# Vandermode/ELD

Measured on AMD Instinct MI355X. Metric: raw megapixels/sec (noise-synth + U-Net step), higher is better.
Workload: dtype f32; 1 GPU; BASELINE.json configs[1]: full ELD noise model (PGRU, SonyA7S2 params) on 4x1424x2128 packed raw + U-Net fp32 train step (fwd, L1, bwd, Adam), 8 frames per GPU; images_per_gpu=8, global_batch=8, parallelism=dp1

## Files before the change

eld_amd/csrc/conv.h:

```cpp
#pragma once
#include "common.h"

typedef float f32x16 __attribute__((ext_vector_type(16)));
typedef float f32x2 __attribute__((ext_vector_type(2)));
typedef __bf16 bf16x2_hw __attribute__((ext_vector_type(2)));

enum ConvMode { CONV_3X3 = 0, CONV_1X1 = 1, CONV_GATHER2X2 = 2 };
enum ConvEpi { EPI_FWD = 0, EPI_CONVT_FWD = 1, EPI_GRAD = 2 };

typedef unsigned short bf16_t;
enum ConvDtype { DT_F32 = 0, DT_BF16 = 1 };

struct ConvArgs {
    const void* in0;
    const void* in1;
    int C0, C1;
    const void* wp;
    int N, H, W;
    int Nout;
    int epi;
    const float* bias;
    int lrelu;
    void* out0;
    void* out1;
// ... 253 lines not shown
    const int full = tiles_x * BH, band = id / full, off = id - band * full;
    int bh = tiles_y - band * BH;
    if (bh > BH) bh = BH;
    tx = off / bh;
    ty = band * BH + (off - tx * bh);
}
int eld_tile_band();
enum { XCD_GEMM = 1, XCD_WGRAD8 = 2, XCD_WGRAD = 4, XCD_X3D = 8, XCD_X3W = 16, XCD_BF16 = 32, XCD_IGEMM = 64 };
int eld_xcd_mask();

struct WgradArgs {
    const void* g;
    int CA;
    const void* x0;
    const void* x1;
    int C0, C1;
    int N, H, W;
    float* part;
    float* bpart;
    float* xbpart;
    int CBp;
    int psplit;
    int tiles_x, tiles_y;
    int vp;
    int dtype;
    int algo;
    int wgrad8;
    int xcd;
    int band;
    const float* amax_g; const float* amax_x0; const float* amax_x1;
};

int launch_wgrad(const WgradArgs& a, int mode, hipStream_t st);
bool wgrad8_shape(int CA, int CBp, int& COB, int& JB, int& TH, int& TWo, bool bf16 = false);
int wgrad8_ntiles(int CA, int CBp, int N, int H, int W, bool bf16);
bool wgradt8_takes(int CA, int CB);
int wgradt8_ntiles(int N, int H, int W);
int launch_wgrad_reduce(const float* part, const float* bpart, float* wgrad, float* bgrad, int psplit, int T, int CA,
                        int CBp, int CBr, hipStream_t st, int bias_n = 0);
```

eld_amd/csrc/conv_wgrad.hip:

```cpp
#include <stdlib.h>
#include "conv.h"

#define TW 32
#define JB 32

typedef __bf16 bf16x8 __attribute__((ext_vector_type(8)));
typedef short s16x4 __attribute__((ext_vector_type(4)));
typedef int i32x4_t __attribute__((ext_vector_type(4)));
typedef _Float16 half8 __attribute__((ext_vector_type(8)));

enum { ALG_F32 = 0, ALG_BFM = 1, ALG_X3 = 2, ALG_H2 = 3 };

template <typename T, int MODE, int WCO, int TH, int ALG>
__global__ __launch_bounds__(256, 2) void wgrad_kernel(const WgradArgs a) {
    constexpr bool BFM = ALG == ALG_BFM, X3 = ALG == ALG_X3, H2 = ALG == ALG_H2;
    static_assert(!(X3 || H2) || sizeof(T) == 4, "x3 / h2: fp32 inputs");
    constexpr int ES = sizeof(T);
    constexpr int EPU = 16 / ES;
    constexpr int LES = X3 ? 6 : (BFM ? 2 : 4);
    constexpr int TAPS = MODE == CONV_3X3 ? 9 : 4;
    constexpr int WPIX = 4 / WCO;
    constexpr int COB = 32 * WCO;
    constexpr int TPIX = TH * TW;
    constexpr int PW = TPIX / WPIX;
// ... 270 lines not shown
                const int row = (i & 3) + 8 * (i >> 2) + 4 * hi;
                a.part[pbase + ((size_t)t * a.CA + i0 + wco * 32 + row) * a.CBp + j0 + m] = H2 ? acc[t][i] * (1.0f / sc_g) * (1.0f / sc_x) : acc[t][i];
            }
        }
    }
    if (a.bpart && jb == 0) {
        red[wave * 64 + lane] = bsum;
        __syncthreads();
        if (tid < COB) {
            const int wc = tid / 32, mm = tid % 32;
            float s = 0.f;
            for (int wp = 0; wp < WPIX; ++wp) s += red[(wp * WCO + wc) * 64 + mm] + red[(wp * WCO + wc) * 64 + 32 + mm];
            a.bpart[(size_t)ps * a.CA + i0 + tid] = H2 ? s * (1.0f / sc_g) : s;
        }
    }
    if constexpr (XSUM) {
        if (xsum_on) {
            __syncthreads();
            float* r = lds;
#pragma unroll
            for (int e = 0; e < EPU; ++e) r[tid * EPU + e] = xs[e];
            __syncthreads();
            if (tid < JB) {
                constexpr int PARTS = JB / EPU;
                const int part = tid / EPU, comp = tid % EPU;
                float s = 0.f;
                for (int k = 0; k < 256 / PARTS; ++k) s += r[(k * PARTS + part) * EPU + comp];
                a.xbpart[(size_t)ps * a.CBp + j0 + tid] = s;
            }
        }
    }
}

template <typename T, int WCO, int WCI, int WPIX, int TH, int TWT, int STREAM = 0>
__global__ __launch_bounds__(512, 2) void wgrad8_kernel(const WgradArgs a) {
    constexpr int ES = sizeof(T), EPU = 16 / ES, NPC = ES == 4 ? 3 : 1, XQ = 32 / EPU;
    static_assert(WCO * WCI * WPIX == 8, "8 waves");
    constexpr int THREADS = 512, TAPS = 9;
    constexpr int COB = 32 * WCO, JBK = 32 * WCI, TPIX = TH * TWT, PW = TPIX / WPIX, KSB = PW / 16;
    static_assert(TWT == 8 || TWT == 16 || TWT == 32, "tile width");
    static_assert(PW % 16 == 0 && PW >= 16, "a wave's pixel slice is a whole number of 16-pixel k-steps");
    constexpr int X_PIX = (TH + 2) * (TWT + 2);
    constexpr int GBLK = TPIX * 32 + (ES == 4 ? 32 : 0);
    constexpr int GPL = GBLK * WCO, XPL = X_PIX * JBK;
    constexpr int G_Q = COB / EPU, G_UNITS = TPIX * G_Q, G_IT = G_UNITS / THREADS;
    static_assert(G_UNITS % THREADS == 0 && THREADS % G_Q == 0, "a thread stages the same channel quad of G in every iteration");
    constexpr int X_UNITS1 = X_PIX * XQ, X_IT = (X_UNITS1 + THREADS - 1) / THREADS;
    extern __shared__ __attribute__((aligned(16))) float lds[];
    bf16_t* ldsG = reinterpret_cast<bf16_t*>(lds);
    bf16_t* ldsX = ldsG + NPC * GPL;

    const int tid = threadIdx.x, lane = tid & 63, wave = tid >> 6;
    const int m = lane & 31, hi = lane >> 5;
    const int wco = wave % WCO, wci = (wave / WCO) % WCI, wpix = wave / (WCO * WCI);
    const int IB = a.CA / COB, JBn = a.CBp / JBK;
    int bid = xcd_block(a.xcd);
    const int jb = bid % JBn; bid /= JBn;
    const int ib = bid % IB;
    const int ps = bid / IB;
    const int i0 = ib * COB, j0 = jb * JBK;
    const bool do_bias = a.bpart != nullptr && jb == 0;

    f32x16 acc[TAPS];
#pragma unroll
    for (int t = 0; t < TAPS; ++t)
#pragma unroll
        for (int i = 0; i < 16; ++i) acc[t][i] = 0.f;
    float4 bsum4 = make_float4(0.f, 0.f, 0.f, 0.f), bsum4b = make_float4(0.f, 0.f, 0.f, 0.f);

    const int ntiles = a.tiles_x * a.tiles_y;
    const int VP = a.vp;
    const bool seam = VP % TH != 0;
    constexpr unsigned OOB = 0xFFFFFFF0u;
    constexpr int G_STEP = THREADS / G_Q;
    const int g_part = tid % G_Q, g_lp0 = tid / G_Q;
    const int g_px0 = g_lp0 % TWT, g_py0 = g_lp0 / TWT;
    const unsigned g_off0 = (unsigned)(g_px0 * a.CA + i0 + g_part * EPU) * (unsigned)ES;
    const int g_lds0 = ((g_part * EPU) >> 5) * GBLK + g_lp0 * 32 + ((g_part * EPU) & 31);
    auto g_pxy = [&](int it, int& dpx, int& dpy) {
        if (G_STEP >= TWT) { dpx = 0; dpy = it * (G_STEP / TWT); }
        else { dpx = (it * G_STEP) % TWT; dpy = (it * G_STEP) / TWT; }
    };
    const int x_part = (int)((unsigned)tid % (unsigned)XQ);
    int x_hyx[X_IT];
#pragma unroll
    for (int it = 0; it < X_IT; ++it) {
        const int hp = (int)((unsigned)(tid + it * THREADS) / (unsigned)XQ);
        const int hy = hp / (TWT + 2);
        x_hyx[it] = (hy << 8) | (hp - hy * (TWT + 2));
    }
    auto x_alive = [&](int it) { return (it + 1) * THREADS <= X_UNITS1 || (int)((unsigned)(tid + it * THREADS) / (unsigned)XQ) < X_PIX; };
    const char* xs[WCI]; int xC[WCI], xc0[WCI];
#pragma unroll
    for (int cb = 0; cb < WCI; ++cb) {
        const int c = j0 + cb * 32;
        if (c < a.C0) { xs[cb] = static_cast<const char*>(a.x0); xC[cb] = a.C0; xc0[cb] = c; }
        else if (c < a.C0 + a.C1) { xs[cb] = static_cast<const char*>(a.x1); xC[cb] = a.C1; xc0[cb] = c - a.C0; }
        else { xs[cb] = nullptr; xC[cb] = 32; xc0[cb] = 0; }
    }
    float4 rg[G_IT], rx[WCI][X_IT];
    const size_t g_img = (size_t)a.H * a.W * a.CA * ES;
    const unsigned g_rowc = (unsigned)(g_py0 * a.W * a.CA) * (unsigned)ES;
    auto load_tile = [&](int tile) {
        int ty, tx;
        band_tile(tile, a.tiles_x, a.tiles_y, a.band, ty, tx);
        const int v0 = ty * TH, x0 = tx * TWT;
        const int img0 = v0 / VP, vrel = v0 - img0 * VP;
        const int wrem = a.W - x0;
        if (!seam || VP - vrel > TH) {
            const __amdgpu_buffer_rsrc_t rs_g = __builtin_amdgcn_make_buffer_rsrc((void*)(static_cast<const char*>(a.g) + (size_t)img0 * g_img), 0, (int)g_img, 0x00020000);
            const int gbase = (vrel * a.W + x0) * a.CA * ES;
#pragma unroll
            for (int it = 0; it < G_IT; ++it) {
                int dpx, dpy;
                g_pxy(it, dpx, dpy);
                const unsigned off = g_off0 + g_rowc + (unsigned)((dpy * a.W + dpx) * a.CA) * (unsigned)ES;
                rg[it] = __builtin_bit_cast(float4, __builtin_amdgcn_raw_buffer_load_b128(rs_g, g_px0 + dpx < wrem ? (int)off : (int)OOB, gbase, 0));
            }
#pragma unroll
            for (int cb = 0; cb < WCI; ++cb) {
                const size_t x_img = (size_t)a.H * a.W * xC[cb] * ES;
                const __amdgpu_buffer_rsrc_t rs_x = __builtin_amdgcn_make_buffer_rsrc((void*)(xs[cb] ? xs[cb] + (size_t)img0 * x_img : nullptr), 0, xs[cb] ? (int)x_img : 0, 0x00020000);
#pragma unroll
                for (int it = 0; it < X_IT; ++it) {
                    const int gy = vrel - 1 + (x_hyx[it] >> 8), gx = x0 - 1 + (x_hyx[it] & 255);
                    const bool ok = x_alive(it) && (unsigned)gy < (unsigned)a.H && (unsigned)gx < (unsigned)a.W;
                    const unsigned off = ok ? (unsigned)((gy * a.W + gx) * xC[cb] + xc0[cb] + x_part * EPU) * (unsigned)ES : OOB;
                    rx[cb][it] = __builtin_bit_cast(float4, __builtin_amdgcn_raw_buffer_load_b128(rs_x, (int)off, 0, 0));
                }
            }
            return;
        }
        const int nimg = a.N - img0 < 2 ? a.N - img0 : 2;
        const int lim0 = a.H - vrel, nxt = VP - vrel;
        const __amdgpu_buffer_rsrc_t rs_g = __builtin_amdgcn_make_buffer_rsrc((void*)(static_cast<const char*>(a.g) + (size_t)img0 * g_img), 0, (int)(g_img * nimg), 0x00020000);
        const unsigned gb0 = (unsigned)((vrel * a.W + x0) * a.CA) * (unsigned)ES;
        const unsigned gb1 = (unsigned)(((a.H - nxt) * a.W + x0) * a.CA) * (unsigned)ES;
#pragma unroll
        for (int it = 0; it < G_IT; ++it) {
            int dpx, dpy;
            g_pxy(it, dpx, dpy);
            const int r = g_py0 + dpy;
            const bool second = r >= nxt;
            const bool ok = (r < lim0 || (second && r - nxt < a.H)) && g_px0 + dpx < wrem;
            const unsigned off = (second ? gb1 : gb0) + g_off0 + g_rowc + (unsigned)((dpy * a.W + dpx) * a.CA) * (unsigned)ES;
            rg[it] = __builtin_bit_cast(float4, __builtin_amdgcn_raw_buffer_load_b128(rs_g, ok ? (int)off : (int)OOB, 0, 0));
        }
#pragma unroll
        for (int cb = 0; cb < WCI; ++cb) {
            const size_t x_img = (size_t)a.H * a.W * xC[cb] * ES;
            const __amdgpu_buffer_rsrc_t rs_x = __builtin_amdgcn_make_buffer_rsrc((void*)(xs[cb] ? xs[cb] + (size_t)img0 * x_img : nullptr), 0, xs[cb] ? (int)(x_img * nimg) : 0, 0x00020000);
#pragma unroll
            for (int it = 0; it < X_IT; ++it) {
                const int r = (x_hyx[it] >> 8) - 1, gx = x0 - 1 + (x_hyx[it] & 255);
                const bool second = r >= nxt;
                const int wrow = second ? a.H + r - nxt : vrel + r;
                const bool rok = second ? r - nxt < a.H : (unsigned)(vrel + r) < (unsigned)a.H;
                const bool ok = x_alive(it) && rok && (unsigned)gx < (unsigned)a.W;
                const unsigned off = ok ? (unsigned)((wrow * a.W + gx) * xC[cb] + xc0[cb] + x_part * EPU) * (unsigned)ES : OOB;
                rx[cb][it] = __builtin_bit_cast(float4, __builtin_amdgcn_raw_buffer_load_b128(rs_x, (int)off, 0, 0));
            }
        }
    };
    auto put3 = [&](bf16_t* d, int plane_elems, const float4& raw) {
        if constexpr (ES == 2) { *reinterpret_cast<float4*>(d) = raw; return; }
        const unsigned x0 = __float_as_uint(raw.x), x1 = __float_as_uint(raw.y), x2 = __float_as_uint(raw.z), x3 = __float_as_uint(raw.w);
        const float r0 = raw.x - __uint_as_float(x0 & 0xFFFF0000u), r1 = raw.y - __uint_as_float(x1 & 0xFFFF0000u);
        const float r2 = raw.z - __uint_as_float(x2 & 0xFFFF0000u), r3 = raw.w - __uint_as_float(x3 & 0xFFFF0000u);
        const unsigned y0 = __float_as_uint(r0), y1 = __float_as_uint(r1), y2 = __float_as_uint(r2), y3 = __float_as_uint(r3);
        const unsigned z0 = __float_as_uint(r0 - __uint_as_float(y0 & 0xFFFF0000u)), z1 = __float_as_uint(r1 - __uint_as_float(y1 & 0xFFFF0000u));
        const unsigned z2 = __float_as_uint(r2 - __uint_as_float(y2 & 0xFFFF0000u)), z3 = __float_as_uint(r3 - __uint_as_float(y3 & 0xFFFF0000u));
        auto hp = [](unsigned lo, unsigned hi_) { return __builtin_amdgcn_perm(hi_, lo, 0x07060302u); };
        *reinterpret_cast<uint2*>(d) = make_uint2(hp(x0, x1), hp(x2, x3));
        *reinterpret_cast<uint2*>(d + plane_elems) = make_uint2(hp(y0, y1), hp(y2, y3));
        *reinterpret_cast<uint2*>(d + 2 * plane_elems) = make_uint2(hp(z0, z1), hp(z2, z3));
    };
    auto store_tile = [&]() {
#pragma unroll
        for (int it = 0; it < G_IT; ++it) {
            put3(ldsG + g_lds0 + it * G_STEP * 32, GPL, rg[it]);
            if (do_bias) {
                if constexpr (ES == 4) { bsum4.x += rg[it].x; bsum4.y += rg[it].y; bsum4.z += rg[it].z; bsum4.w += rg[it].w; }
                else {
                    const uint4 q = __builtin_bit_cast(uint4, rg[it]);
                    const float4 lo = unpack_bf4(make_uint2(q.x, q.y)), hi4 = unpack_bf4(make_uint2(q.z, q.w));
                    bsum4.x += lo.x; bsum4.y += lo.y; bsum4.z += lo.z; bsum4.w += lo.w;
                    bsum4b.x += hi4.x; bsum4b.y += hi4.y; bsum4b.z += hi4.z; bsum4b.w += hi4.w;
                }
            }
        }
#pragma unroll
        for (int cb = 0; cb < WCI; ++cb)
#pragma unroll
            for (int it = 0; it < X_IT; ++it)
                if (x_alive(it)) put3(ldsX + (cb * X_PIX + (int)((unsigned)(tid + it * THREADS) / (unsigned)XQ)) * 32 + x_part * EPU, XPL, rx[cb][it]);
    };

    const int gi = lane & 15, gg = lane >> 4;
    constexpr bool ROWSHARE = STREAM == 2;
    static_assert(!ROWSHARE || (NPC == 3 && TWT == 8 && WPIX == 1 && TH % 2 == 0), "row-shared fragments: fp32, 8-pixel-wide tiles, one pixel slice");
    constexpr int HS = TH / 2;
    const int lq0 = ROWSHARE ? HS * TWT * hi + (gi >> 2) : wpix * PW + 8 * hi + (gi >> 2);
    const int pyq = lq0 / TWT, pxq = lq0 - pyq * TWT;
    const bf16_t* gq = ldsG + wco * GBLK + lq0 * 32 + (gg & 1) * 16 + (gi & 3) * 4;
    const bf16_t* xq = ldsX + (wci * X_PIX + pyq * (TWT + 2) + pxq) * 32 + (gg & 1) * 16 + (gi & 3) * 4;
    auto tr8 = [](const bf16_t* p0) {
        const s16x4 lo = __builtin_amdgcn_ds_read_tr16_b64_v4i16((__attribute__((address_space(3))) s16x4*)p0);
        const s16x4 hi4 = __builtin_amdgcn_ds_read_tr16_b64_v4i16((__attribute__((address_space(3))) s16x4*)(p0 + 4 * 32));
        return __builtin_bit_cast(bf16x8, __builtin_shufflevector(lo, hi4, 0, 1, 2, 3, 4, 5, 6, 7));
    };

    if (ps < ntiles) load_tile(ps);
    for (int tile = ps; tile < ntiles; tile += a.psplit) {
        __syncthreads();
        store_tile();
        __syncthreads();
        if (tile + a.psplit < ntiles) load_tile(tile + a.psplit);
        if constexpr (ROWSHARE) {
            constexpr int GI[6] = {0, 1, 2, 0, 1, 0};
            constexpr int XI[6] = {2, 1, 0, 1, 0, 0};
            constexpr int NU = (HS + 2) * 3;
            bf16x8 gr[3][3], xf[2][3];
            auto readG = [&](int s_, bf16x8 (&g3)[3]) {
#pragma unroll
                for (int pc = 0; pc < 3; ++pc) g3[pc] = tr8(gq + pc * GPL + s_ * TWT * 32);
            };
            auto readF = [&](int a_, int kx, bf16x8 (&x3)[3]) {
#pragma unroll
                for (int pc = 0; pc < 3; ++pc) x3[pc] = tr8(xq + pc * XPL + (a_ * (TWT + 2) + kx) * 32);
            };
            readG(0, gr[0]);
            readF(0, 0, xf[0]);
#pragma unroll
            for (int u = 0; u < NU; ++u) {
                const int a_ = u / 3, kx = u % 3;
                if (u + 1 < NU) readF((u + 1) / 3, (u + 1) % 3, xf[(u + 1) & 1]);
                __builtin_amdgcn_sched_barrier(0);
#pragma unroll
// ... 21 lines not shown
#pragma unroll
                for (int pc = 0; pc < 3; ++pc) g3[pc] = tr8(gq + pc * GPL + ks * 16 * 32);
            };
            auto readX = [&](int ks, int t, bf16x8 (&x3)[3]) {
                const int lrel = ks * 16, dy0 = lrel / TWT, dxp = lrel - dy0 * TWT;
                const int xoff = (dy0 + t / 3) * (TWT + 2) + dxp + t % 3;
#pragma unroll
                for (int pc = 0; pc < 3; ++pc) x3[pc] = tr8(xq + pc * XPL + xoff * 32);
            };
            readG(0, ga[0]);
            readX(0, 0, xb[0]);
#pragma unroll
            for (int b = 0; b < NBLK; ++b) {
                const int ks = b / TAPS, t = b % TAPS;
                if (b + 1 < NBLK) {
                    const int ks1 = (b + 1) / TAPS, t1 = (b + 1) % TAPS;
                    readX(ks1, t1, xb[(b + 1) & 1]);
                    if (ks1 != ks) readG(ks1, ga[ks1 & 1]);
                }
                __builtin_amdgcn_sched_barrier(0);
#pragma unroll
                for (int q = 0; q < 6; ++q) acc[t] = __builtin_amdgcn_mfma_f32_32x32x16_bf16(ga[ks & 1][GI[q]], xb[b & 1][XI[q]], acc[t], 0, 0, 0);
                __builtin_amdgcn_sched_barrier(0);
            }
        } else
#pragma unroll
        for (int ks = 0; ks < KSB; ++ks) {
            const int lrel = ks * 16;
            const int dy0 = lrel / TWT, dxp = lrel - dy0 * TWT;
            bf16x8 ga[NPC];
#pragma unroll
            for (int pc = 0; pc < NPC; ++pc) ga[pc] = tr8(gq + pc * GPL + lrel * 32);
#pragma unroll
            for (int t0 = 0; t0 < TAPS; t0 += 3) {
                bf16x8 xb[3][NPC];
#pragma unroll
                for (int tt = 0; tt < 3; ++tt) {
                    const int xoff = (dy0 + t0 / 3) * (TWT + 2) + dxp + tt;
#pragma unroll
                    for (int pc = 0; pc < NPC; ++pc) xb[tt][pc] = tr8(xq + pc * XPL + xoff * 32);
                }
                if constexpr (NPC == 3) {
                    constexpr int GI[6] = {0, 1, 2, 0, 1, 0};
                    constexpr int XI[6] = {2, 1, 0, 1, 0, 0};
#pragma unroll
                    for (int q = 0; q < 6; ++q)
#pragma unroll
                        for (int tt = 0; tt < 3; ++tt)
                            acc[t0 + tt] = __builtin_amdgcn_mfma_f32_32x32x16_bf16(ga[GI[q]], xb[tt][XI[q]], acc[t0 + tt], 0, 0, 0);
                } else {
#pragma unroll
                    for (int tt = 0; tt < 3; ++tt) acc[t0 + tt] = __builtin_amdgcn_mfma_f32_32x32x16_bf16(ga[0], xb[tt][0], acc[t0 + tt], 0, 0, 0);
                }
                __builtin_amdgcn_sched_barrier(0);
            }
        }
    }

    __syncthreads();
    float* red = lds;
    const size_t pbase = (size_t)ps * TAPS * a.CA * a.CBp;
    const int wt = wci * WCO + wco;
#pragma unroll
    for (int t = 0; t < TAPS; ++t) {
        if (WPIX > 1) {
            if (wpix > 0) {
#pragma unroll
                for (int i = 0; i < 16; ++i) red[(((wpix - 1) * (WCO * WCI) + wt) * 16 + i) * 64 + lane] = acc[t][i];
            }
            __syncthreads();
            if (wpix == 0) {
                for (int w = 0; w < WPIX - 1; ++w)
#pragma unroll
                    for (int i = 0; i < 16; ++i) acc[t][i] += red[((w * (WCO * WCI) + wt) * 16 + i) * 64 + lane];
            }
            __syncthreads();
        }
        if (wpix == 0) {
#pragma unroll
            for (int i = 0; i < 16; ++i) {
                const int row = (i & 3) + 8 * (i >> 2) + 4 * hi;
                a.part[pbase + ((size_t)t * a.CA + i0 + wco * 32 + row) * a.CBp + j0 + wci * 32 + m] = acc[t][i];
            }
        }
    }
    if (do_bias) {
        __syncthreads();
        if constexpr (ES == 4) reinterpret_cast<float4*>(red)[tid] = bsum4;
        else { reinterpret_cast<float4*>(red)[2 * tid] = bsum4; reinterpret_cast<float4*>(red)[2 * tid + 1] = bsum4b; }
        __syncthreads();
        if (tid < COB) {
            const int q = tid / EPU, comp = tid % EPU;
            float s_ = 0.f;
            for (int k = 0; k < THREADS / G_Q; ++k) s_ += red[(q + k * G_Q) * EPU + comp];
            a.bpart[(size_t)ps * a.CA + i0 + tid] = s_;
        }
    }
}

__device__ __forceinline__ void wg_dma16(i32x4_t rsrc, unsigned voff, unsigned lds_dst) {
    unsigned keep;
    asm volatile("s_nop 4\n\ts_mov_b32 %0, m0\n\ts_mov_b32 m0, %3\n\ts_nop 0\n\tbuffer_load_dwordx4 %1, %2, 0 offen lds\n\ts_mov_b32 m0, %0"
                 : "=&s"(keep) : "v"(voff), "s"(rsrc), "s"(lds_dst) : "memory");
}

template <int WCO, int WCI, int WPIX, int TH, int TWT>
__global__ __launch_bounds__(512, 2) void wgrad8d_kernel(const WgradArgs a) {
    static_assert(WCO * WCI * WPIX == 8, "8 waves");
    static_assert(TWT == 8 || TWT == 16 || TWT == 32, "tile width");
    constexpr int WAVES = 8, THREADS = 512, TAPS = 9;
    constexpr int COB = 32 * WCO, JBK = 32 * WCI, TPIX = TH * TWT, PW = TPIX / WPIX, KSB = PW / 16;
    static_assert(PW % 16 == 0 && PW >= 16, "a wave's pixel slice is a whole number of 16-pixel k-steps");
    constexpr int HW = TWT + 2, X_PIX = (TH + 2) * HW;
    static_assert((TPIX * 4) % 64 == 0, "a block of G is whole DMA pieces");
    constexpr int GB_PIECES = TPIX * 4 / 64, XB_PIECES = (X_PIX * 4 + 63) / 64;
// ... 339 lines not shown
        if (tid < JBK) {
            const int cb = tid >> 5, c = tid & 31, quad = c >> 2, comp = c & 3;
            float s_ = 0.f;
            for (int k = 0; k < THREADS / 8; ++k) s_ += reinterpret_cast<const float*>(&r[cb * THREADS + quad + 8 * k])[comp];
            a.xbpart[(size_t)ps * a.CBp + j0 + tid] = s_;
        }
    }
}

bool wgradt8_takes(int CA, int CB) {
    static const int on = [] { const char* e = getenv("ELD_WGRADT8"); return e ? atoi(e) : 1; }();
    return on && CA % 128 == 0 && CB % 64 == 0;
}
int wgradt8_ntiles(int N, int H, int W) { return ((W + 7) / 8) * ((H + 7) / 8) * N; }

static int launch_wt8(WgradArgs a, hipStream_t st) {
    eld_note_conv_kernel("wgradt8");
    a.xcd = eld_xcd_mask() & XCD_WGRAD8;
    a.band = eld_tile_band();
    a.tiles_x = (a.W + 7) / 8;
    a.tiles_y = (a.H + 7) / 8;
    const size_t lds_bytes = (size_t)(3 * 4 * (64 * 32 + 32) + 3 * 2 * 256 * 32) * 2;
    const long long blocks = (long long)(a.CA / 128) * (a.CBp / 64) * a.psplit;
    if (blocks <= 0) return 0;
    if ((size_t)4 * a.H * a.W * a.C0 * 4 >= 0xFFFFFFF0ull || (size_t)a.H * a.W * a.CA * 4 >= 0xFFFFFFF0ull) return ELD_ENOTSUP;
    auto kern = wgradt8_kernel<0>;
    static EldAttrOnce once;
    { const int rc = once.ensure(kern, lds_bytes); if (rc) return rc; }
    ELD_LAUNCH(kern, dim3((unsigned)blocks), dim3(512), lds_bytes, st, a);
    ELD_LAUNCH_CHECK();
    return 0;
}

bool wgrad8_shape(int CA, int CBp, int& COB, int& JBK, int& TH, int& TWo, bool bf16) {
    if (CA % 32 || CBp % 32) return false;
    TWo = 32;
    if (CA % 128 == 0 && CBp % 64 == 0) { COB = 128; JBK = 64; TH = 2; }
    else if (CA % 64 == 0 && CBp % 64 == 0) { COB = 64; JBK = 64; TH = 2; }
    else if (CA % 64 == 0) { COB = 64; JBK = 32; TH = 4; }
    else if (CBp % 64 == 0) { COB = 32; JBK = 64; TH = 4; }
    else { COB = 32; JBK = 32; TH = 4; }
    if (bf16) TH = 8;
    if (bf16 && wgrad8_dma() && COB == 128) { TH = 16; TWo = 8; return true; }
    if (COB == 128) { TH = TH * 4; TWo = 8; }
    return true;
}

int wgrad8_ntiles(int CA, int CBp, int N, int H, int W, bool bf16) {
    int COB, JBK, TH, TWo;
    if (!wgrad8_shape(CA, CBp, COB, JBK, TH, TWo, bf16)) return 0;
    const int VP = vrow_pitch(N, H, TH);
    return ((W + TWo - 1) / TWo) * ((vrow_extent(N, H, VP) + TH - 1) / TH);
}

template <typename T, int WCO, int WCI, int WPIX, int TH, int TWT, int STREAM = 0>
static int launch_w8(WgradArgs a, hipStream_t st) {
    a.xcd = eld_xcd_mask() & XCD_WGRAD8;
    a.band = eld_tile_band();
    constexpr int COB = 32 * WCO, JBK = 32 * WCI;
    eld_note_conv_variant(sizeof(T) == 2 ? "wgrad8<bf16>" : (COB == 128 ? "wgrad8<f32,128x64>" : (COB == 64 ? (JBK == 64 ? "wgrad8<f32,64x64>" : "wgrad8<f32,64x32>")
                                                                                                     : (JBK == 64 ? "wgrad8<f32,32x64>" : "wgrad8<f32,32x32>"))),
                          STREAM == 1 ? "stream" : (STREAM == 2 ? "rowshare" : nullptr));
    a.vp = vrow_pitch(a.N, a.H, TH);
    a.tiles_x = (a.W + TWT - 1) / TWT;
    a.tiles_y = (vrow_extent(a.N, a.H, a.vp) + TH - 1) / TH;
    size_t lds_bytes = (size_t)((TH * TWT * 32 + (sizeof(T) == 4 ? 32 : 0)) * (COB / 32) + (TH + 2) * (TWT + 2) * JBK) * (sizeof(T) == 4 ? 6 : 2);
    const size_t red_bytes = (size_t)7 * 16 * 64 * sizeof(float) * 1;
    if (lds_bytes < red_bytes) lds_bytes = red_bytes;
    const long long blocks = (long long)(a.CA / COB) * (a.CBp / JBK) * a.psplit;
    if (blocks <= 0) return 0;
    auto kern = wgrad8_kernel<T, WCO, WCI, WPIX, TH, TWT, STREAM>;
    static EldAttrOnce once;
    { const int rc = once.ensure(kern, lds_bytes); if (rc) return rc; }
    ELD_LAUNCH(kern, dim3((unsigned)blocks), dim3(512), lds_bytes, st, a);
    ELD_LAUNCH_CHECK();
    return 0;
}

template <int WCO, int WCI, int WPIX, int TH, int TWT>
static int launch_w8d(WgradArgs a, hipStream_t st) {
    eld_note_conv_kernel("wgrad8d");
    a.xcd = eld_xcd_mask() & XCD_WGRAD8;
    a.band = eld_tile_band();
    constexpr int COB = 32 * WCO, JBK = 32 * WCI;
    a.vp = vrow_pitch(a.N, a.H, TH);
    a.tiles_x = (a.W + TWT - 1) / TWT;
    a.tiles_y = (vrow_extent(a.N, a.H, a.vp) + TH - 1) / TH;
    constexpr int PIECES = WCO * (TH * TWT * 4 / 64) + WCI * (((TH + 2) * (TWT + 2) * 4 + 63) / 64);
    size_t lds_bytes = (size_t)2 * PIECES * 1024;
    const size_t red_bytes = (size_t)7 * 16 * 64 * sizeof(float);
    if (lds_bytes < red_bytes) lds_bytes = red_bytes;
    const long long blocks = (long long)(a.CA / COB) * (a.CBp / JBK) * a.psplit;
    if (blocks <= 0) return 0;
    auto kern = wgrad8d_kernel<WCO, WCI, WPIX, TH, TWT>;
    static EldAttrOnce once;
    { const int rc = once.ensure(kern, lds_bytes); if (rc) return rc; }
    ELD_LAUNCH(kern, dim3((unsigned)blocks), dim3(512), lds_bytes, st, a);
    ELD_LAUNCH_CHECK();
    return 0;
}

static int launch_wgrad8(const WgradArgs& a, hipStream_t st) {
    const bool bf16 = a.dtype == DT_BF16;
    const size_t es = bf16 ? 2 : 4;
    int COB, JBK, TH, TWo;
    if (!wgrad8_shape(a.CA, a.CBp, COB, JBK, TH, TWo, bf16)) return ELD_ENOTSUP;
    if ((a.C0 % 32) || (a.C1 % 32)) return ELD_ENOTSUP;
    const size_t win = a.N > 1 ? 2 : 1;
    if ((size_t)a.H * a.W * a.CA * es * win >= 0xFFFFFFF0ull || (size_t)a.H * a.W * (a.C0 > a.C1 ? a.C0 : a.C1) * es * win >= 0xFFFFFFF0ull) return ELD_ENOTSUP;
    if (bf16 && wgrad8_dma() && COB == 128) {
        return launch_w8d<4, 2, 1, 16, 8>(a, st);
    }
    if (bf16) {
        if (COB == 128) return launch_w8<bf16_t, 4, 2, 1, 32, 8>(a, st);
        if (COB == 64 && JBK == 64) return launch_w8<bf16_t, 2, 2, 2, 8, 32>(a, st);
        if (COB == 64) return launch_w8<bf16_t, 2, 1, 4, 8, 32>(a, st);
        if (JBK == 64) return launch_w8<bf16_t, 1, 2, 4, 8, 32>(a, st);
        return launch_w8<bf16_t, 1, 1, 8, 8, 32>(a, st);
    }
    static const int stream = [] { const char* e = getenv("ELD_WG8_STREAM"); return e ? atoi(e) : 0; }();
    static const int rowshare = [] { const char* e = getenv("ELD_WG8_ROWSHARE"); return e ? atoi(e) : 0; }();
    if (COB == 128 && rowshare) return launch_w8<float, 4, 2, 1, 8, 8, 2>(a, st);
    if (COB == 128) return (stream & 1) ? launch_w8<float, 4, 2, 1, 8, 8, 1>(a, st) : launch_w8<float, 4, 2, 1, 8, 8>(a, st);
    if (stream & 2) {
        if (COB == 64 && JBK == 64) return launch_w8<float, 2, 2, 2, 2, 32, 1>(a, st);
        if (COB == 64) return launch_w8<float, 2, 1, 4, 4, 32, 1>(a, st);
        if (JBK == 64) return launch_w8<float, 1, 2, 4, 4, 32, 1>(a, st);
        return launch_w8<float, 1, 1, 8, 4, 32, 1>(a, st);
    }
    if (COB == 64 && JBK == 64) return launch_w8<float, 2, 2, 2, 2, 32>(a, st);
    if (COB == 64) return launch_w8<float, 2, 1, 4, 4, 32>(a, st);
    if (JBK == 64) return launch_w8<float, 1, 2, 4, 4, 32>(a, st);
    return launch_w8<float, 1, 1, 8, 4, 32>(a, st);
}

template <typename T, int MODE, int WCO, int TH, int ALG = ALG_F32>
static int launch_w(WgradArgs a, hipStream_t st) {
    eld_note_conv_variant(sizeof(T) == 2 ? (MODE == CONV_3X3 ? "wgrad<bf16>" : "wgrad<bf16,gather>") : (MODE == CONV_3X3 ? "wgrad<f32>" : "wgrad<f32,gather>"),
                          (sizeof(T) == 2 && ALG == ALG_F32) ? "f32mma" : nullptr);
    a.xcd = eld_xcd_mask() & XCD_WGRAD;
    constexpr int COB = 32 * WCO;
    constexpr int X_PIX = MODE == CONV_3X3 ? (TH + 2) * (TW + 2) : 4 * TH * TW;
    a.tiles_x = (a.W + TW - 1) / TW;
    a.tiles_y = (a.H + TH - 1) / TH;
    constexpr int GROWS = TH * TW + ((ALG == ALG_X3 || ALG == ALG_H2) ? 1 : 0);
    size_t lds_bytes = (size_t)(GROWS * COB + X_PIX * JB) * (ALG == ALG_X3 ? 6 : (ALG == ALG_BFM ? 2 : 4));
    const size_t red_bytes = (size_t)4 * 16 * 64 * sizeof(float);
    if (lds_bytes < red_bytes) lds_bytes = red_bytes;
    const long long blocks = (long long)(a.CA / COB) * (a.CBp / JB) * a.psplit;
    if (blocks <= 0) return 0;
    auto kern = wgrad_kernel<T, MODE, WCO, TH, ALG>;
    static EldAttrOnce once;
    { const int rc = once.ensure(kern, lds_bytes); if (rc) return rc; }
    ELD_LAUNCH(kern, dim3((unsigned)blocks), dim3(256), lds_bytes, st, a);
    ELD_LAUNCH_CHECK();
    return 0;
}

int launch_wgrad(const WgradArgs& a, int mode, hipStream_t st) {
    if (a.CA % 32 || a.CBp % 32 || a.C0 % 4 || a.C1 % 4 || a.psplit < 1) return ELD_EINVAL;
    if (a.C1 > 0 && a.C0 % 32) return ELD_EINVAL;
    const bool c64 = a.CA % 64 == 0;
    if (a.dtype == DT_BF16) {
        if (a.C0 % 8 || a.C1 % 8) return ELD_EINVAL;
        if (mode == CONV_3X3 && a.wgrad8) {
            const int rc = launch_wgrad8(a, st);
// ... 110 lines not shown
```

eld_amd/csrc/unet.hip:

```cpp
#include <mutex>
#include <unordered_map>
#include <math.h>
#include "unet_misc.h"

namespace {

constexpr int NLEV = 5;
inline int chan(int l) { return 32 << l; }

struct LayerDef {
    int kind;
    int cin, cout;
    size_t w_off, b_off;
};

enum {
    L_E0A = 0, L_E0B, L_E1A, L_E1B, L_E2A, L_E2B, L_E3A, L_E3B, L_E4A, L_E4B,
    L_UP3, L_D3A, L_D3B, L_UP2, L_D2A, L_D2B, L_UP1, L_D1A, L_D1B, L_UP0, L_D0A, L_D0B, L_HEAD, NLAYERS
};

size_t build_layers(int in_ch, int out_ch, LayerDef* L) {
    int k = 0;
    for (int l = 0; l < NLEV; ++l) {
        L[k++] = {0, l == 0 ? in_ch : chan(l - 1), chan(l), 0, 0};
// ... 10 lines not shown
        const size_t taps = L[i].kind == 0 ? 9 : (L[i].kind == 1 ? 4 : 1);
        L[i].w_off = off; off += (size_t)L[i].cin * L[i].cout * taps;
        L[i].b_off = off; off += L[i].cout;
    }
    return off;
}

inline size_t align_up(size_t x, size_t a) { return (x + a - 1) / a * a; }

int choose_psplit(int groups, int ntiles) {
    int ps = 512 / groups;
    if (ps < 1) ps = 1;
    if (ps > ntiles) ps = ntiles;
    if (ps < 1) ps = 1;
    return ps;
}

struct WgradGeom { int T, CA, CBp, groups, ntiles, psplit, w8; size_t floats; };

WgradGeom wgrad_geom(int mode, int CA, int CB, int N, int H, int W, int algo) {
    WgradGeom g;
    g.T = mode == CONV_3X3 ? 9 : 4;
    g.CA = CA;
    g.CBp = (CB + 31) / 32 * 32;
    g.w8 = 0;
    int cob8, jb8, th8, tw8;
    if ((algo == 1 || algo == 3) && mode == CONV_3X3 && CB % 32 == 0 && wgrad8_shape(CA, g.CBp, cob8, jb8, th8, tw8, algo == 3)) {
        g.w8 = 1;
        g.groups = (CA / cob8) * (g.CBp / jb8);
        g.ntiles = wgrad8_ntiles(CA, g.CBp, N, H, W, algo == 3);
        int ps = 256 / g.groups;
        if (ps > g.ntiles) ps = g.ntiles;
        g.psplit = ps < 1 ? 1 : ps;
        g.floats = (size_t)g.psplit * ((size_t)g.T * CA * g.CBp + CA);
        return g;
    }
    if (algo == 1 && mode == CONV_GATHER2X2 && CB == g.CBp && wgradt8_takes(CA, CB)) {
        g.w8 = 1;
        g.groups = (CA / 128) * (g.CBp / 64);
        g.ntiles = wgradt8_ntiles(N, H, W);
        int ps = 256 / g.groups;
        if (ps > g.ntiles) ps = g.ntiles;
        g.psplit = ps < 1 ? 1 : ps;
        g.floats = (size_t)g.psplit * ((size_t)g.T * CA * g.CBp + CA);
        return g;
    }
    const int COB = (CA % 64 == 0) ? 64 : 32;
    const int TH = mode == CONV_3X3 ? 4 : 2;
    g.groups = (CA / COB) * (g.CBp / 32);
    g.ntiles = ((W + 31) / 32) * ((H + TH - 1) / TH) * N;
    g.psplit = choose_psplit(g.groups, g.ntiles);
    g.floats = (size_t)g.psplit * ((size_t)g.T * CA * g.CBp + CA);
    return g;
}

struct Amax { const float* in0 = nullptr; const float* in1 = nullptr; const float* w = nullptr; float* out0 = nullptr; float* out1 = nullptr; };
thread_local Amax g_am;
struct KPart { float* p = nullptr; size_t floats = 0; };
thread_local KPart g_kp;
struct KPartScope { KPart prev; KPartScope(float* p, size_t n) : prev(g_kp) { g_kp.p = p; g_kp.floats = n; } ~KPartScope() { g_kp = prev; } };
thread_local int g_algo = -1;
struct AlgoScope { int prev; explicit AlgoScope(int a) : prev(g_algo) { g_algo = resolve_algo(a); } ~AlgoScope() { g_algo = prev; } };
inline void take_amax(ConvArgs& a) { a.algo = g_algo; a.amax_in0 = g_am.in0; a.amax_in1 = g_am.in1; a.amax_w = g_am.w; a.amax_out0 = g_am.out0; a.amax_out1 = g_am.out1; g_am = Amax(); }
inline void take_amax(WgradArgs& a) { a.algo = g_algo; a.amax_g = g_am.in0; a.amax_x0 = g_am.w; a.amax_x1 = g_am.in1; g_am = Amax(); }
enum { S_W = 0, S_X = 23, S_EA = 24, S_EB = 29, S_UP = 34, S_DA = 38, S_DB = 42, S_GA = 46, S_GB = 47, S_SKIP = 48, S_COUNT = 64 };
int conv_fwd(const float* in0, int C0, const float* in1, int C1, const float* wp, const float* bias, float* out, int N, int H, int W,
             int Cout, int lrelu, hipStream_t st, float* pool_out = nullptr, unsigned* codes_out = nullptr, unsigned* pool_codes_out = nullptr) {
// ... 1087 lines not shown
```

Measured before the change: 734.9 raw MPix/s.

## Split wgrad8 fp32 kernel taps across 12 waves by kernel row

Adds a WTAP=3 variant of the 8-wave weight-gradient kernel in which each of three wave groups handles one row of the 3x3 kernel (three taps), giving 12 waves per block. Each wave now holds three tap accumulators instead of nine, which frees registers, and the pixel tiles become taller (TH=8, sometimes TW=16). It is the default for fp32 shapes with COB<128. Staging G now needs guarded partial iterations, and the workspace sizing in unet is widened to cover either tiling. The cost is more waves per block sharing LDS, a different tile count and psplit, and extra bounds checks.

Measured after the change: 742.1 raw MPix/s (median of 6 runs). About the same (+1.0%).

```diff
diff --git a/eld_amd/csrc/conv.h b/eld_amd/csrc/conv.h
--- a/eld_amd/csrc/conv.h
+++ b/eld_amd/csrc/conv.h
@@ -309,8 +309,8 @@
 };
 
 int launch_wgrad(const WgradArgs& a, int mode, hipStream_t st);
-bool wgrad8_shape(int CA, int CBp, int& COB, int& JB, int& TH, int& TWo, bool bf16 = false);
-int wgrad8_ntiles(int CA, int CBp, int N, int H, int W, bool bf16);
+bool wgrad8_shape(int CA, int CBp, int& COB, int& JB, int& TH, int& TWo, bool bf16 = false, int rows = -1, int* wtap = nullptr);
+int wgrad8_ntiles(int CA, int CBp, int N, int H, int W, bool bf16, int rows = -1);
 bool wgradt8_takes(int CA, int CB);
 int wgradt8_ntiles(int N, int H, int W);
 int launch_wgrad_reduce(const float* part, const float* bpart, float* wgrad, float* bgrad, int psplit, int T, int CA,
diff --git a/eld_amd/csrc/conv_wgrad.hip b/eld_amd/csrc/conv_wgrad.hip
--- a/eld_amd/csrc/conv_wgrad.hip
+++ b/eld_amd/csrc/conv_wgrad.hip
@@ -326,19 +326,22 @@
     }
 }
 
-template <typename T, int WCO, int WCI, int WPIX, int TH, int TWT, int STREAM = 0>
-__global__ __launch_bounds__(512, 2) void wgrad8_kernel(const WgradArgs a) {
+template <typename T, int WCO, int WCI, int WPIX, int TH, int TWT, int STREAM = 0, int WTAP = 1>
+__global__ __launch_bounds__(512 * (WTAP == 3 ? 3 : 2) / 2, WTAP == 3 ? 3 : 2) void wgrad8_kernel(const WgradArgs a) {
     constexpr int ES = sizeof(T), EPU = 16 / ES, NPC = ES == 4 ? 3 : 1, XQ = 32 / EPU;
-    static_assert(WCO * WCI * WPIX == 8, "8 waves");
-    constexpr int THREADS = 512, TAPS = 9;
+    static_assert(WTAP == 1 || WTAP == 3, "all nine taps per wave, or one kernel row");
+    static_assert(WCO * WCI * WPIX * WTAP == (WTAP == 3 ? 12 : 8), "8 waves, or 12 with the kernel-row split");
+    static_assert(WTAP == 1 || (STREAM == 0 && ES == 4), "kernel-row split: fp32 inputs, default main loop");
+    constexpr int THREADS = 64 * WCO * WCI * WPIX * WTAP, TAPS = 9, NT = TAPS / WTAP;
     constexpr int COB = 32 * WCO, JBK = 32 * WCI, TPIX = TH * TWT, PW = TPIX / WPIX, KSB = PW / 16;
     static_assert(TWT == 8 || TWT == 16 || TWT == 32, "tile width");
     static_assert(PW % 16 == 0 && PW >= 16, "a wave's pixel slice is a whole number of 16-pixel k-steps");
     constexpr int X_PIX = (TH + 2) * (TWT + 2);
     constexpr int GBLK = TPIX * 32 + (ES == 4 ? 32 : 0);
     constexpr int GPL = GBLK * WCO, XPL = X_PIX * JBK;
-    constexpr int G_Q = COB / EPU, G_UNITS = TPIX * G_Q, G_IT = G_UNITS / THREADS;
-    static_assert(G_UNITS % THREADS == 0 && THREADS % G_Q == 0, "a thread stages the same channel quad of G in every iteration");
+    constexpr int G_Q = COB / EPU, G_UNITS = TPIX * G_Q, G_IT = (G_UNITS + THREADS - 1) / THREADS;
+    constexpr bool G_EXACT = G_UNITS % THREADS == 0;
+    static_assert((G_EXACT || WTAP == 3) && THREADS % G_Q == 0, "a thread stages the same channel quad of G in every iteration");
     constexpr int X_UNITS1 = X_PIX * XQ, X_IT = (X_UNITS1 + THREADS - 1) / THREADS;
     extern __shared__ __attribute__((aligned(16))) float lds[];
     bf16_t* ldsG = reinterpret_cast<bf16_t*>(lds);
@@ -346,7 +349,8 @@
 
     const int tid = threadIdx.x, lane = tid & 63, wave = tid >> 6;
     const int m = lane & 31, hi = lane >> 5;
-    const int wco = wave % WCO, wci = (wave / WCO) % WCI, wpix = wave / (WCO * WCI);
+    const int wco = wave % WCO, wci = (wave / WCO) % WCI, wpix = WTAP == 3 ? (wave / (WCO * WCI)) % WPIX : wave / (WCO * WCI);
+    const int kyb = WTAP == 3 ? wave / (WCO * WCI * WPIX) : 0;
     const int IB = a.CA / COB, JBn = a.CBp / JBK;
     int bid = xcd_block(a.xcd);
     const int jb = bid % JBn; bid /= JBn;
@@ -355,9 +359,9 @@
     const int i0 = ib * COB, j0 = jb * JBK;
     const bool do_bias = a.bpart != nullptr && jb == 0;
 
-    f32x16 acc[TAPS];
-#pragma unroll
-    for (int t = 0; t < TAPS; ++t)
+    f32x16 acc[NT];
+#pragma unroll
+    for (int t = 0; t < NT; ++t)
 #pragma unroll
         for (int i = 0; i < 16; ++i) acc[t][i] = 0.f;
     float4 bsum4 = make_float4(0.f, 0.f, 0.f, 0.f), bsum4b = make_float4(0.f, 0.f, 0.f, 0.f);
@@ -395,6 +399,14 @@
     float4 rg[G_IT], rx[WCI][X_IT];
     const size_t g_img = (size_t)a.H * a.W * a.CA * ES;
     const unsigned g_rowc = (unsigned)(g_py0 * a.W * a.CA) * (unsigned)ES;
+    static_assert(G_STEP % TWT == 0 || TWT % G_STEP == 0, "a G pass is whole tile rows, or divides one");
+    auto g_alive = [&](int it) { return G_EXACT || (it + 1) * G_STEP <= TPIX || g_lp0 + it * G_STEP < TPIX; };
+    auto g_at = [&](int it, int& px, int& r, unsigned& off) {
+        int dpx, dpy;
+        g_pxy(it, dpx, dpy);
+        px = g_px0 + dpx; r = g_py0 + dpy;
+        off = g_off0 + g_rowc + (unsigned)((dpy * a.W + dpx) * a.CA) * (unsigned)ES;
+    };
     auto load_tile = [&](int tile) {
         int ty, tx;
         band_tile(tile, a.tiles_x, a.tiles_y, a.band, ty, tx);
@@ -406,10 +418,16 @@
             const int gbase = (vrel * a.W + x0) * a.CA * ES;
 #pragma unroll
             for (int it = 0; it < G_IT; ++it) {
-                int dpx, dpy;
-                g_pxy(it, dpx, dpy);
-                const unsigned off = g_off0 + g_rowc + (unsigned)((dpy * a.W + dpx) * a.CA) * (unsigned)ES;
-                rg[it] = __builtin_bit_cast(float4, __builtin_amdgcn_raw_buffer_load_b128(rs_g, g_px0 + dpx < wrem ? (int)off : (int)OOB, gbase, 0));
+                if constexpr (WTAP == 1) {
+                    int dpx, dpy;
+                    g_pxy(it, dpx, dpy);
+                    const unsigned off = g_off0 + g_rowc + (unsigned)((dpy * a.W + dpx) * a.CA) * (unsigned)ES;
+                    rg[it] = __builtin_bit_cast(float4, __builtin_amdgcn_raw_buffer_load_b128(rs_g, g_px0 + dpx < wrem ? (int)off : (int)OOB, gbase, 0));
+                } else {
+                    int px, r; unsigned off;
+                    g_at(it, px, r, off);
+                    rg[it] = __builtin_bit_cast(float4, __builtin_amdgcn_raw_buffer_load_b128(rs_g, g_alive(it) && px < wrem ? (int)off : (int)OOB, gbase, 0));
+                }
             }
 #pragma unroll
             for (int cb = 0; cb < WCI; ++cb) {
@@ -432,13 +450,22 @@
         const unsigned gb1 = (unsigned)(((a.H - nxt) * a.W + x0) * a.CA) * (unsigned)ES;
 #pragma unroll
         for (int it = 0; it < G_IT; ++it) {
-            int dpx, dpy;
-            g_pxy(it, dpx, dpy);
-            const int r = g_py0 + dpy;
-            const bool second = r >= nxt;
-            const bool ok = (r < lim0 || (second && r - nxt < a.H)) && g_px0 + dpx < wrem;
-            const unsigned off = (second ? gb1 : gb0) + g_off0 + g_rowc + (unsigned)((dpy * a.W + dpx) * a.CA) * (unsigned)ES;
-            rg[it] = __builtin_bit_cast(float4, __builtin_amdgcn_raw_buffer_load_b128(rs_g, ok ? (int)off : (int)OOB, 0, 0));
+            if constexpr (WTAP == 1) {
+                int dpx, dpy;
+                g_pxy(it, dpx, dpy);
+                const int r = g_py0 + dpy;
+                const bool second = r >= nxt;
+                const bool ok = (r < lim0 || (second && r - nxt < a.H)) && g_px0 + dpx < wrem;
+                const unsigned off = (second ? gb1 : gb0) + g_off0 + g_rowc + (unsigned)((dpy * a.W + dpx) * a.CA) * (unsigned)ES;
+                rg[it] = __builtin_bit_cast(float4, __builtin_amdgcn_raw_buffer_load_b128(rs_g, ok ? (int)off : (int)OOB, 0, 0));
+            } else {
+                int px, r; unsigned offr;
+                g_at(it, px, r, offr);
+                const bool second = r >= nxt;
+                const bool ok = g_alive(it) && (r < lim0 || (second && r - nxt < a.H)) && px < wrem;
+                const unsigned off = (second ? gb1 : gb0) + offr;
+                rg[it] = __builtin_bit_cast(float4, __builtin_amdgcn_raw_buffer_load_b128(rs_g, ok ? (int)off : (int)OOB, 0, 0));
+            }
         }
 #pragma unroll
         for (int cb = 0; cb < WCI; ++cb) {
@@ -472,7 +499,7 @@
     auto store_tile = [&]() {
 #pragma unroll
         for (int it = 0; it < G_IT; ++it) {
-            put3(ldsG + g_lds0 + it * G_STEP * 32, GPL, rg[it]);
+            if (g_alive(it)) put3(ldsG + g_lds0 + it * G_STEP * 32, GPL, rg[it]);
             if (do_bias) {
                 if constexpr (ES == 4) { bsum4.x += rg[it].x; bsum4.y += rg[it].y; bsum4.z += rg[it].z; bsum4.w += rg[it].w; }
                 else {
@@ -497,7 +524,7 @@
     const int lq0 = ROWSHARE ? HS * TWT * hi + (gi >> 2) : wpix * PW + 8 * hi + (gi >> 2);
     const int pyq = lq0 / TWT, pxq = lq0 - pyq * TWT;
     const bf16_t* gq = ldsG + wco * GBLK + lq0 * 32 + (gg & 1) * 16 + (gi & 3) * 4;
-    const bf16_t* xq = ldsX + (wci * X_PIX + pyq * (TWT + 2) + pxq) * 32 + (gg & 1) * 16 + (gi & 3) * 4;
+    const bf16_t* xq = ldsX + (wci * X_PIX + (pyq + kyb) * (TWT + 2) + pxq) * 32 + (gg & 1) * 16 + (gi & 3) * 4;
     auto tr8 = [](const bf16_t* p0) {
         const s16x4 lo = __builtin_amdgcn_ds_read_tr16_b64_v4i16((__attribute__((address_space(3))) s16x4*)p0);
         const s16x4 hi4 = __builtin_amdgcn_ds_read_tr16_b64_v4i16((__attribute__((address_space(3))) s16x4*)(p0 + 4 * 32));
@@ -585,7 +612,7 @@
 #pragma unroll
             for (int pc = 0; pc < NPC; ++pc) ga[pc] = tr8(gq + pc * GPL + lrel * 32);
 #pragma unroll
-            for (int t0 = 0; t0 < TAPS; t0 += 3) {
+            for (int t0 = 0; t0 < NT; t0 += 3) {
                 bf16x8 xb[3][NPC];
 #pragma unroll
                 for (int tt = 0; tt < 3; ++tt) {
@@ -613,27 +640,29 @@
     __syncthreads();
     float* red = lds;
     const size_t pbase = (size_t)ps * TAPS * a.CA * a.CBp;
-    const int wt = wci * WCO + wco;
-#pragma unroll
-    for (int t = 0; t < TAPS; ++t) {
+    constexpr int WT = WCO * WCI * WTAP;
+    const int wt = (kyb * WCI + wci) * WCO + wco;
+#pragma unroll
+    for (int t = 0; t < NT; ++t) {
         if (WPIX > 1) {
             if (wpix > 0) {
 #pragma unroll
-                for (int i = 0; i < 16; ++i) red[(((wpix - 1) * (WCO * WCI) + wt) * 16 + i) * 64 + lane] = acc[t][i];
+                for (int i = 0; i < 16; ++i) red[(((wpix - 1) * WT + wt) * 16 + i) * 64 + lane] = acc[t][i];
             }
             __syncthreads();
             if (wpix == 0) {
                 for (int w = 0; w < WPIX - 1; ++w)
 #pragma unroll
-                    for (int i = 0; i < 16; ++i) acc[t][i] += red[((w * (WCO * WCI) + wt) * 16 + i) * 64 + lane];
+                    for (int i = 0; i < 16; ++i) acc[t][i] += red[((w * WT + wt) * 16 + i) * 64 + lane];
             }
             __syncthreads();
         }
         if (wpix == 0) {
+            const int tap = kyb * NT + t;
 #pragma unroll
             for (int i = 0; i < 16; ++i) {
                 const int row = (i & 3) + 8 * (i >> 2) + 4 * hi;
-                a.part[pbase + ((size_t)t * a.CA + i0 + wco * 32 + row) * a.CBp + j0 + wci * 32 + m] = acc[t][i];
+                a.part[pbase + ((size_t)tap * a.CA + i0 + wco * 32 + row) * a.CBp + j0 + wci * 32 + m] = acc[t][i];
             }
         }
     }
@@ -1039,7 +1068,14 @@
     return 0;
 }
 
-bool wgrad8_shape(int CA, int CBp, int& COB, int& JBK, int& TH, int& TWo, bool bf16) {
+static int wgrad8_stream() {
+    static const int stream = [] { const char* e = getenv("ELD_WG8_STREAM"); return e ? atoi(e) : 0; }();
+    return stream;
+}
+static bool wgrad8_rows(int rows) { return rows < 0 ? !(debug_kernel_mask(-1) & 512) && !(wgrad8_stream() & 2) : rows != 0; }
+
+bool wgrad8_shape(int CA, int CBp, int& COB, int& JBK, int& TH, int& TWo, bool bf16, int rows, int* wtap) {
+    if (wtap) *wtap = 1;
     if (CA % 32 || CBp % 32) return false;
     TWo = 32;
     if (CA % 128 == 0 && CBp % 64 == 0) { COB = 128; JBK = 64; TH = 2; }
@@ -1047,39 +1083,51 @@
     else if (CA % 64 == 0) { COB = 64; JBK = 32; TH = 4; }
     else if (CBp % 64 == 0) { COB = 32; JBK = 64; TH = 4; }
     else { COB = 32; JBK = 32; TH = 4; }
+    if (!bf16 && COB < 128 && wgrad8_rows(rows)) {
+        if (wtap) *wtap = 3;
+        TH = 8;
+        if (COB == 64 || JBK == 64) TWo = 16;
+        return true;
+    }
     if (bf16) TH = 8;
     if (bf16 && wgrad8_dma() && COB == 128) { TH = 16; TWo = 8; return true; }
     if (COB == 128) { TH = TH * 4; TWo = 8; }
     return true;
 }
 
-int wgrad8_ntiles(int CA, int CBp, int N, int H, int W, bool bf16) {
+int wgrad8_ntiles(int CA, int CBp, int N, int H, int W, bool bf16, int rows) {
     int COB, JBK, TH, TWo;
-    if (!wgrad8_shape(CA, CBp, COB, JBK, TH, TWo, bf16)) return 0;
+    if (!wgrad8_shape(CA, CBp, COB, JBK, TH, TWo, bf16, rows)) return 0;
     const int VP = vrow_pitch(N, H, TH);
     return ((W + TWo - 1) / TWo) * ((vrow_extent(N, H, VP) + TH - 1) / TH);
 }
 
-template <typename T, int WCO, int WCI, int WPIX, int TH, int TWT, int STREAM = 0>
-static int launch_w8(WgradArgs a, hipStream_t st) {
+template <typename T, int WCO, int WCI, int WPIX, int TH, int TWT, int STREAM = 0, int WTAP = 1>
+static int launch_w8(WgradArgs a, hipStream_t st, const char* routed = nullptr) {
+    {
+        int cob, jbk, th, two, wtap;
+        if (!wgrad8_shape(a.CA, a.CBp, cob, jbk, th, two, sizeof(T) == 2, WTAP == 3, &wtap) || th != TH || two != TWT || wtap != WTAP) return ELD_EINVAL;
+    }
     a.xcd = eld_xcd_mask() & XCD_WGRAD8;
     a.band = eld_tile_band();
     constexpr int COB = 32 * WCO, JBK = 32 * WCI;
     eld_note_conv_variant(sizeof(T) == 2 ? "wgrad8<bf16>" : (COB == 128 ? "wgrad8<f32,128x64>" : (COB == 64 ? (JBK == 64 ? "wgrad8<f32,64x64>" : "wgrad8<f32,64x32>")
                                                                                                      : (JBK == 64 ? "wgrad8<f32,32x64>" : "wgrad8<f32,32x32>"))),
-                          STREAM == 1 ? "stream" : (STREAM == 2 ? "rowshare" : nullptr));
+                          STREAM == 1 ? "stream" : (STREAM == 2 ? "rowshare" : routed));
     a.vp = vrow_pitch(a.N, a.H, TH);
     a.tiles_x = (a.W + TWT - 1) / TWT;
     a.tiles_y = (vrow_extent(a.N, a.H, a.vp) + TH - 1) / TH;
     size_t lds_bytes = (size_t)((TH * TWT * 32 + (sizeof(T) == 4 ? 32 : 0)) * (COB / 32) + (TH + 2) * (TWT + 2) * JBK) * (sizeof(T) == 4 ? 6 : 2);
-    const size_t red_bytes = (size_t)7 * 16 * 64 * sizeof(float) * 1;
+    constexpr int THREADS = 64 * WCO * WCI * WPIX * WTAP;
+    constexpr size_t red_tiles = (size_t)(WPIX - 1) * WCO * WCI * WTAP * 16 * 64 * sizeof(float), red_bias = (size_t)THREADS * (sizeof(T) == 4 ? 16 : 32);
+    constexpr size_t red_bytes = red_tiles > red_bias ? red_tiles : red_bias;
     if (lds_bytes < red_bytes) lds_bytes = red_bytes;
     const long long blocks = (long long)(a.CA / COB) * (a.CBp / JBK) * a.psplit;
     if (blocks <= 0) return 0;
-    auto kern = wgrad8_kernel<T, WCO, WCI, WPIX, TH, TWT, STREAM>;
+    auto kern = wgrad8_kernel<T, WCO, WCI, WPIX, TH, TWT, STREAM, WTAP>;
     static EldAttrOnce once;
     { const int rc = once.ensure(kern, lds_bytes); if (rc) return rc; }
-    ELD_LAUNCH(kern, dim3((unsigned)blocks), dim3(512), lds_bytes, st, a);
+    ELD_LAUNCH(kern, dim3((unsigned)blocks), dim3(THREADS), lds_bytes, st, a);
     ELD_LAUNCH_CHECK();
     return 0;
 }
@@ -1110,8 +1158,8 @@
 static int launch_wgrad8(const WgradArgs& a, hipStream_t st) {
     const bool bf16 = a.dtype == DT_BF16;
     const size_t es = bf16 ? 2 : 4;
-    int COB, JBK, TH, TWo;
-    if (!wgrad8_shape(a.CA, a.CBp, COB, JBK, TH, TWo, bf16)) return ELD_ENOTSUP;
+    int COB, JBK, TH, TWo, wtap;
+    if (!wgrad8_shape(a.CA, a.CBp, COB, JBK, TH, TWo, bf16, -1, &wtap)) return ELD_ENOTSUP;
     if ((a.C0 % 32) || (a.C1 % 32)) return ELD_ENOTSUP;
     const size_t win = a.N > 1 ? 2 : 1;
     if ((size_t)a.H * a.W * a.CA * es * win >= 0xFFFFFFF0ull || (size_t)a.H * a.W * (a.C0 > a.C1 ? a.C0 : a.C1) * es * win >= 0xFFFFFFF0ull) return ELD_ENOTSUP;
@@ -1125,7 +1173,7 @@
         if (JBK == 64) return launch_w8<bf16_t, 1, 2, 4, 8, 32>(a, st);
         return launch_w8<bf16_t, 1, 1, 8, 8, 32>(a, st);
     }
-    static const int stream = [] { const char* e = getenv("ELD_WG8_STREAM"); return e ? atoi(e) : 0; }();
+    const int stream = wgrad8_stream();
     static const int rowshare = [] { const char* e = getenv("ELD_WG8_ROWSHARE"); return e ? atoi(e) : 0; }();
     if (COB == 128 && rowshare) return launch_w8<float, 4, 2, 1, 8, 8, 2>(a, st);
     if (COB == 128) return (stream & 1) ? launch_w8<float, 4, 2, 1, 8, 8, 1>(a, st) : launch_w8<float, 4, 2, 1, 8, 8>(a, st);
@@ -1135,10 +1183,19 @@
         if (JBK == 64) return launch_w8<float, 1, 2, 4, 4, 32, 1>(a, st);
         return launch_w8<float, 1, 1, 8, 4, 32, 1>(a, st);
     }
-    if (COB == 64 && JBK == 64) return launch_w8<float, 2, 2, 2, 2, 32>(a, st);
-    if (COB == 64) return launch_w8<float, 2, 1, 4, 4, 32>(a, st);
-    if (JBK == 64) return launch_w8<float, 1, 2, 4, 4, 32>(a, st);
-    return launch_w8<float, 1, 1, 8, 4, 32>(a, st);
+    if (wtap == 3) {
+        if (COB == 64 && JBK == 64) return launch_w8<float, 2, 2, 1, 8, 16, 0, 3>(a, st);
+        if (COB == 64) return launch_w8<float, 2, 1, 2, 8, 16, 0, 3>(a, st);
+        if (JBK == 64) return launch_w8<float, 1, 2, 2, 8, 16, 0, 3>(a, st);
+        return launch_w8<float, 1, 1, 4, 8, 32, 0, 3>(a, st);
+    }
+    int wt1 = 1;
+    { int c, j, t, w; wgrad8_shape(a.CA, a.CBp, c, j, t, w, false, 1, &wt1); }
+    const char* routed = wt1 == 3 ? "8wave" : nullptr;
+    if (COB == 64 && JBK == 64) return launch_w8<float, 2, 2, 2, 2, 32>(a, st, routed);
+    if (COB == 64) return launch_w8<float, 2, 1, 4, 4, 32>(a, st, routed);
+    if (JBK == 64) return launch_w8<float, 1, 2, 4, 4, 32>(a, st, routed);
+    return launch_w8<float, 1, 1, 8, 4, 32>(a, st, routed);
 }
 
 template <typename T, int MODE, int WCO, int TH, int ALG = ALG_F32>
diff --git a/eld_amd/csrc/unet.hip b/eld_amd/csrc/unet.hip
--- a/eld_amd/csrc/unet.hip
+++ b/eld_amd/csrc/unet.hip
@@ -66,7 +66,12 @@
         int ps = 256 / g.groups;
         if (ps > g.ntiles) ps = g.ntiles;
         g.psplit = ps < 1 ? 1 : ps;
-        g.floats = (size_t)g.psplit * ((size_t)g.T * CA * g.CBp + CA);
+        int nt8 = wgrad8_ntiles(CA, g.CBp, N, H, W, algo == 3, 0);
+        if (nt8 < g.ntiles) nt8 = g.ntiles;
+        int psmax = 256 / g.groups;
+        if (psmax > nt8) psmax = nt8;
+        if (psmax < g.psplit) psmax = g.psplit;
+        g.floats = (size_t)psmax * ((size_t)g.T * CA * g.CBp + CA);
         return g;
     }
     if (algo == 1 && mode == CONV_GATHER2X2 && CB == g.CBp && wgradt8_takes(CA, CB)) {
```
